# taufikxu/MOG-ASR

Hardware: AMD Instinct MI355X
Metric: images/sec/node AIR train step, Multi-MNIST 50×50 max_steps=3, 1/2/4/8 GPU (higher is better)
Workload: dtype fp32; 1 GPU; AIR baseline train step (training_air_original.py AIRModel, fp32), per-GPU batch 8192 (configs[1] batch); model=AIR (LSTM 256, VAE 784-512-256-50, heads 64), global_batch=8192, per_gpu_batch=8192, canvas=50x50, max_steps=3, data_dependent_steps_would_be=3, parallelism=dp1

## Files before the change

include/mog_air.h:

```cpp
#ifndef MOG_AIR_H
#define MOG_AIR_H

#ifdef __cplusplus
extern "C" {
#endif

#define MOG_ERR_INVALID 1001

int mog_gemm_f32(int batch, const float* const* A, const float* const* B, float* const* C,
                 const float* const* bias, const float* const* Cin, float* const* Cpre,
                 const float* const* aux, float* const* colsum, int M, int N, int K, int lda,
                 int ldb, int ldc, int ldaux, int transA, int transB, int epi, float aux_scale,
                 int splitk, void* stream);

int mog_gemm_f32_x3_tn(const float* A, const float* B, float* C, float* colsum, int M, int N,
                       int K, int lda, int ldb, int ldc, int splitk, float* work, long work_elems,
                       void* stream);

int mog_split3_bf16(const float* src, int rows, int cols, int ld_src, void* dst, int ld_dst,
                    long piece_stride, void* stream);
int mog_split3_sum_bf16(const float* src, int nsum, long sum_stride, int rows, int cols,
                        int ld_src, void* dst, int ld_dst, long piece_stride, void* stream);
int mog_gemm_x3p_tn(const void* A3, long sa, const void* B3, long sb, float* C, float* colsum,
                    int M, int N, int K, int lda, int ldb, int ldc, int splitk, int npieces,
// ... 1 lines not shown

int mog_build_id(char* out, int cap);

int mog_gemm_f32_wgrad_group(const long long* table, int nprob, void* stream);

long mog_wgrad_tn_work_elems(int nprob, const int* dims, int nsplit);
int mog_wgrad_tn_bf16(int nprob, const void* const* X, const void* const* dY, float* const* out,
                      float* const* colsum, const int* dims, int K, int nsplit, float* work,
                      long work_elems, void* stream);
int mog_wgrad_tn_x3(int nprob, const float* const* X, const float* const* dY, float* const* out,
                    float* const* colsum, const int* dims, int K, int nsplit, float* work,
                    long work_elems, void* stream);

int mog_gemm_x3_nt(const float* A, const void* B3, long sb, float* C, const float* aux, int M,
                   int N, int K, int lda, int ldb, int ldc, int ldaux, int epi, void* stream);

int mog_gemm_f32_sigmoid_philox(const float* A, const float* B, float* C, const float* bias,
                                int M, int N, int K, int lda, int ldb, int ldc, float scale,
                                unsigned long long seed, unsigned long long offset,
                                void* stream);
int mog_gemm_f32_kseg(int nseg, const float* const* A, const float* const* B, float* C,
                      const float* bias, const float* Cin, int M, int N, int kseg, int lda,
                      int ldb, int ldc, int transA, int transB, int epi, void* stream);
int mog_gemm_f32_kseg_group(int nprob, const int* nseg, const float* const* A,
                            const float* const* B, float* const* C, const float* const* Cin, int M,
                            int N, int kseg, int lda, int ldb, int ldc, int transB, void* stream);

int mog_stn_forward(const float* U, int N, int Hin, int Win, const float* theta, int Hout,
                    int Wout, void* out, const float* z, const float* mask, int mode,
                    void* stream);
// ... 238 lines not shown
```

mog-asr_amd/csrc/air_cell.hip:

```cpp
#include <algorithm>

#include "mog_common.h"

namespace {

struct LstmFwd {
  const float* G;
  const float* bias;
  const float* c_prev;
  float* c_out;
  float* h_out;
};

__device__ __forceinline__ void lstm_fwd_body(const LstmFwd& a, int B, int H, long idx) {
#pragma clang fp contract(off)
  if (idx >= (long)B * H) return;
  const int b = idx / H, u = idx - (long)b * H;
  const float* g = a.G + (size_t)b * 4 * H;
  float gi = g[u], gj = g[H + u], gf = g[2 * H + u], go = g[3 * H + u];
  if (a.bias) {
    const float* bias = a.bias;
    gi = gi + bias[u]; gj = gj + bias[H + u]; gf = gf + bias[2 * H + u]; go = go + bias[3 * H + u];
  }
  const float c0 = a.c_prev ? a.c_prev[idx] : 0.0f;
// ... 27 lines not shown
};

__device__ __forceinline__ void lstm_bwd_body(const LstmBwd& a, int B, int H, long idx) {
  if (idx >= (long)B * H) return;
  const int b = idx / H, u = idx - (long)b * H;
  const float* g = a.G + (size_t)b * 4 * H;
  const float* bp = a.bias ? a.bias : a.G;
  const float* cp = a.c_prev ? a.c_prev : a.c_cur;
  const float* dp = a.dc ? a.dc : a.dh;
  float* sp = a.dGsum ? a.dGsum + (size_t)b * 4 * H : a.dG + (size_t)b * 4 * H;
  float gi = g[u], gj = g[H + u], gf = g[2 * H + u], go = g[3 * H + u];
  const float bi = bp[u], bj = bp[H + u], bf = bp[2 * H + u], bo = bp[3 * H + u];
  const float cpv = cp[idx], ctv = a.c_cur[idx], dcv = dp[idx];
  float dhv = a.dh[idx];
  if (a.nparts > 0) {
    float pv[4];
#pragma unroll
    for (int j = 0; j < 4; ++j) pv[j] = j < a.nparts ? a.dh_parts[j * a.part_stride + idx] : 0.0f;
#pragma unroll
    for (int j = 0; j < 4; ++j)
      if (j < a.nparts) dhv = dhv + pv[j];
  }
  const float s0 = sp[u], s1 = sp[H + u], s2 = sp[2 * H + u], s3 = sp[3 * H + u];
  if (a.bias) {
    gi = gi + bi; gj = gj + bj; gf = gf + bf; go = go + bo;
  }
  const float si = mog_sigmoidf(gi), tj = mog_tanhf(gj), sf = mog_sigmoidf(gf + 1.0f);
  const float so = mog_sigmoidf(go);
  const float c0 = a.c_prev ? cpv : 0.0f;
  const float tc = mog_tanhf(ctv);
  const float dct = (a.dc ? dcv : 0.0f) + dhv * so * (1.0f - tc * tc);
  const float dgo = dhv * tc * so * (1.0f - so);
  const float dgf = dct * c0 * sf * (1.0f - sf);
  const float dgi = dct * tj * si * (1.0f - si);
  const float dgj = dct * si * (1.0f - tj * tj);
// ... 796 lines not shown
                                      float* dG, float* dc_prev, float* dGsum, int B, int H,
                                      void* stream) {
  MOG_CHECK_ARG(G && c_cur && dh && dG && B >= 0 && H > 0);
  if (B == 0) return 0;
  lstm_bwd_kernel<<<mog_cdiv((long)B * H, 256), 256, 0, mog_stream(stream)>>>(
      LstmBwd{G, bias, c_prev, c_cur, dh, dc, dG, dc_prev, dGsum}, B, H);
  MOG_LAUNCH_RET();
}

extern "C" int mog_lstm_cell_backward_parts(const float* G, const float* bias,
                                            const float* c_prev, const float* c_cur,
                                            const float* dh, const float* dh_parts, int nparts,
                                            long part_stride, const float* dc, float* dG,
                                            float* dc_prev, float* dGsum, int B, int H,
                                            void* stream) {
  MOG_CHECK_ARG(G && c_cur && dh && dG && B >= 0 && H > 0 && nparts >= 0 && nparts <= 4);
  MOG_CHECK_ARG(nparts == 0 || (dh_parts && part_stride >= (long)B * H));
  if (B == 0) return 0;
  LstmBwd a{G, bias, c_prev, c_cur, dh, dc, dG, dc_prev, dGsum};
  a.dh_parts = dh_parts;
  a.nparts = nparts;
  a.part_stride = part_stride;
  lstm_bwd_kernel<<<mog_cdiv((long)B * H, 256), 256, 0, mog_stream(stream)>>>(a, B, H);
  MOG_LAUNCH_RET();
}

extern "C" int mog_lstm_cell_forward_pair(const float* const* cells, int B, int H, void* stream) {
  MOG_CHECK_ARG(cells && B >= 0 && H > 0);
  const float* const* a = cells;
  const float* const* b = cells + 5;
  MOG_CHECK_ARG(a[0] && a[3] && a[4] && b[0] && b[3] && b[4]);
// ... 351 lines not shown
```

mog-asr_amd/csrc/gemm_x3.hip:

```cpp
#include <cstdlib>
#include <type_traits>

#include "mog_common.h"
#include "x3_split.h"

namespace {

typedef __bf16 bf16x8 __attribute__((ext_vector_type(8)));
typedef __bf16 bf16x4 __attribute__((ext_vector_type(4)));
typedef __attribute__((address_space(3))) bf16x4 lds_bf16x4;
typedef unsigned int u32x4 __attribute__((ext_vector_type(4)));

constexpr int BM = 128, BN = 128, BK = 32;
constexpr int LDR = BM;
constexpr int PIECE = BK * LDR;
constexpr int STAGE = 6 * PIECE;
constexpr int NL = (BM * BK / 4) / 256;

__device__ __forceinline__ int xcd_remap(int orig, int nwg) {
  const int xcd = orig & 7, q = nwg >> 3, r = nwg & 7;
  return (xcd < r ? xcd * (q + 1) : r * (q + 1) + (xcd - r) * q) + (orig >> 3);
}

__device__ __forceinline__ int tsw(int r) { return ((r & 3) << 2) | (((r >> 3) & 1) << 4); }
// ... 321 lines not shown
    float v = W[e];
    for (int s = 1; s < nsplit; ++s) v += W[s * MN + e];
    C[(size_t)(e / N) * ldc + e % N] += v;
  }
}

void splitk_reduce(const X3Args& D, hipStream_t s) {
  const long n4 = ((long)D.M * D.N + 3) / 4;
  const long nt = n4 > D.N ? n4 : (long)D.N;
  const bool vec = D.N % 4 == 0 && D.ldc % 4 == 0 && (reinterpret_cast<uintptr_t>(D.C) & 15) == 0;
  splitk_reduce_kernel<<<dim3((unsigned)((nt + 255) / 256)), 256, 0, s>>>(
      D.work, D.nsplit, D.C, D.M, D.N, D.ldc, vec, D.colsum);
}

constexpr int NT_LDK = BK + 16;
constexpr int NT_PIECE = BM * NT_LDK;
constexpr int NT_STAGE = 6 * NT_PIECE;
constexpr int NT_NLA = (BM * BK / 4) / 256;
constexpr int NT_NLB = (BN * BK / 8) / 256;

struct X3NtArgs {
  const float* A;
  const __bf16* B3;
  long sb;
  float* C;
  const float* aux;
  int M, N, K, lda, ldb, ldc, ldaux, nx, ny, epi;
};

__device__ __forceinline__ float xt_dpp1(float v) {
  return __int_as_float(__builtin_amdgcn_mov_dpp(__float_as_int(v), 0xB1, 0xF, 0xF, false));
}
__device__ __forceinline__ float xt_dpp2(float v) {
  return __int_as_float(__builtin_amdgcn_mov_dpp(__float_as_int(v), 0x4E, 0xF, 0xF, false));
}
__device__ __forceinline__ floatx4 xt_quad_transpose(const floatx4& a, int lane) {
  const int e = lane & 3;
  float r0 = a[0], r1 = a[1], r2 = a[2], r3 = a[3];
  {
    const bool hi = (e & 2) != 0;
    const float t0 = xt_dpp2(hi ? r0 : r2), t1 = xt_dpp2(hi ? r1 : r3);
    if (hi) { r0 = t0; r1 = t1; } else { r2 = t0; r3 = t1; }
  }
  {
    const bool od = (e & 1) != 0;
    const float t0 = xt_dpp1(od ? r0 : r1), t1 = xt_dpp1(od ? r2 : r3);
    if (od) { r0 = t0; r2 = t1; } else { r1 = t0; r3 = t1; }
  }
  return floatx4{r0, r1, r2, r3};
}

template <int EPI>
__global__ __launch_bounds__(256, 2) void gemm_x3_nt_kernel(X3NtArgs D) {
  __shared__ __attribute__((aligned(16))) __bf16 lds[NT_STAGE];
  const int nwg = gridDim.x;
  const int wg = xcd_remap(blockIdx.x, nwg);
  const int bx = wg % D.nx, by = wg / D.nx;
  const int m0 = by * BM, n0 = bx * BN;
  const int t = threadIdx.x, lane = t & 63, w = t >> 6;
  const int wm = (w >> 1) * 64, wn = (w & 1) * 64;
  const int M = D.M, N = D.N, K = D.K;
  const int ar = t >> 3, ak = (t & 7) * 4;
  const int br = t >> 2, bk = (t & 3) * 8;
  floatx4 acc[4][4];
#pragma unroll
  for (int mi = 0; mi < 4; ++mi)
#pragma unroll
    for (int ni = 0; ni < 4; ++ni) acc[mi][ni] = floatx4{0.f, 0.f, 0.f, 0.f};
  u32x4 ra[NT_NLA];
  u32x4 rb[3][NT_NLB];
  const int arows = min(M - m0, BM);
  const __amdgpu_buffer_rsrc_t arsc = __builtin_amdgcn_make_buffer_rsrc(
      const_cast<float*>(D.A) + (size_t)m0 * D.lda, 0,
      (M - m0 > BM ? BM * D.lda : (arows - 1) * D.lda + K) * 4, 0x00020000);
  __amdgpu_buffer_rsrc_t brsc[3];
#pragma unroll
  for (int p = 0; p < 3; ++p)
    brsc[p] = __builtin_amdgcn_make_buffer_rsrc(const_cast<__bf16*>(D.B3) + (size_t)p * D.sb, 0,
                                                ((N - 1) * D.ldb + K) * 2, 0x00020000);
  int avo[NT_NLA], bvo[NT_NLB];
#pragma unroll
  for (int i = 0; i < NT_NLA; ++i) avo[i] = ((ar + 32 * i) * D.lda + ak) * 4;
#pragma unroll
  for (int i = 0; i < NT_NLB; ++i) bvo[i] = ((n0 + br + 64 * i) * D.ldb + bk) * 2;
  constexpr int OOB = (int)0x80000000u;
  auto load_tiles = [&](int k0) {
    const bool ak_in = k0 + ak < K, bk_in = k0 + bk < K;
#pragma unroll
    for (int i = 0; i < NT_NLA; ++i)
      ra[i] = __builtin_amdgcn_raw_buffer_load_b128(arsc, ak_in ? avo[i] : OOB, k0 * 4, 0);
#pragma unroll
    for (int i = 0; i < NT_NLB; ++i)
#pragma unroll
      for (int p = 0; p < 3; ++p)
        rb[p][i] = __builtin_amdgcn_raw_buffer_load_b128(brsc[p], bk_in ? bvo[i] : OOB, k0 * 2, 0);
  };
  auto store_tiles = [&]() {
#pragma unroll
    for (int i = 0; i < NT_NLA; ++i) {
      const int o = (ar + 32 * i) * NT_LDK + ak;
      u32x2 p0, p1, p2;
      split4(float4{__uint_as_float(ra[i][0]), __uint_as_float(ra[i][1]),
                    __uint_as_float(ra[i][2]), __uint_as_float(ra[i][3])},
             p0, p1, p2);
      *reinterpret_cast<u32x2*>(lds + 0 * NT_PIECE + o) = p0;
      *reinterpret_cast<u32x2*>(lds + 1 * NT_PIECE + o) = p1;
      *reinterpret_cast<u32x2*>(lds + 2 * NT_PIECE + o) = p2;
    }
#pragma unroll
    for (int i = 0; i < NT_NLB; ++i) {
      const int o = (br + 64 * i) * NT_LDK + bk;
#pragma unroll
      for (int p = 0; p < 3; ++p) *reinterpret_cast<u32x4*>(lds + (3 + p) * NT_PIECE + o) = rb[p][i];
    }
  };
  const int g = lane >> 4, li = lane & 15;
  auto frag = [&](int piece, int row) -> bf16x8 {
    return *reinterpret_cast<const bf16x8*>(lds + piece * NT_PIECE + (row + li) * NT_LDK + 8 * g);
  };
  auto compute = [&]() {
    bf16x8 b[3][4];
#pragma unroll
    for (int p = 0; p < 3; ++p)
#pragma unroll
      for (int i = 0; i < 4; ++i) b[p][i] = frag(3 + p, wn + 16 * i);
    auto pass = [&](const bf16x8 (&x)[4], const bf16x8 (&y)[4]) {
#pragma unroll
      for (int mi = 0; mi < 4; ++mi)
#pragma unroll
        for (int ni = 0; ni < 4; ++ni)
          acc[mi][ni] = __builtin_amdgcn_mfma_f32_16x16x32_bf16(x[mi], y[ni], acc[mi][ni], 0, 0, 0);
    };
#pragma unroll
    for (int pa = 2; pa >= 0; --pa) {
      bf16x8 a[4];
#pragma unroll
      for (int i = 0; i < 4; ++i) a[i] = frag(pa, wm + 16 * i);
#pragma unroll
      for (int pb = 2 - pa; pb >= 0; --pb) pass(a, b[pb]);
    }
  };
  const int nk = (K + BK - 1) / BK;
  load_tiles(0);
  for (int it = 0; it < nk; ++it) {
    store_tiles();
    if (it + 1 < nk) load_tiles((it + 1) * BK);
    __syncthreads();
    compute();
    __syncthreads();
  }
  u32x4 xq[4][4];
  if constexpr (EPI == 1) {
    const __amdgpu_buffer_rsrc_t xr = __builtin_amdgcn_make_buffer_rsrc(
        const_cast<float*>(D.aux) + (size_t)m0 * D.ldaux, 0,
        (M - m0 > BM ? BM * D.ldaux : (arows - 1) * D.ldaux + N) * 4, 0x00020000);
#pragma unroll
    for (int mi = 0; mi < 4; ++mi)
#pragma unroll
      for (int ni = 0; ni < 4; ++ni)
        xq[mi][ni] = __builtin_amdgcn_raw_buffer_load_b128(
            xr, ((wm + mi * 16 + g * 4 + (li & 3)) * D.ldaux + n0 + wn + ni * 16 + (li & ~3)) * 4,
            0, 0);
  }
#pragma unroll
  for (int mi = 0; mi < 4; ++mi)
#pragma unroll
    for (int ni = 0; ni < 4; ++ni) {
      const floatx4 v = xt_quad_transpose(acc[mi][ni], lane);
      const int row = m0 + wm + mi * 16 + g * 4 + (li & 3);
      const int col = n0 + wn + ni * 16 + (li & ~3);
      float o[4] = {v[0], v[1], v[2], v[3]};
      if (EPI == 1) {
#pragma unroll
        for (int q = 0; q < 4; ++q) o[q] = v[q] * -mog_expm1f(-__uint_as_float(xq[mi][ni][q]));
      }
      if (row < M && col < N)
        *reinterpret_cast<float4*>(D.C + (size_t)row * D.ldc + col) = make_float4(o[0], o[1], o[2], o[3]);
    }
}

}

extern "C" int mog_split3_bf16(const float* src, int rows, int cols, int ld_src, void* dst,
                               int ld_dst, long piece_stride, void* stream) {
  MOG_CHECK_ARG(src && dst && rows >= 0 && cols >= 0 && cols % 4 == 0 && ld_src % 4 == 0 &&
                ld_dst % 4 == 0 && ld_dst >= cols && ld_src >= cols && piece_stride % 4 == 0 &&
                piece_stride >= (long)rows * ld_dst && al16(src) && al16(dst));
  const long n = (long)rows * (ld_dst / 4);
  if (n == 0) return 0;
  split3_kernel<<<dim3((unsigned)((n + 255) / 256)), 256, 0, mog_stream(stream)>>>(
      src, rows, cols, ld_src, reinterpret_cast<__bf16*>(dst), ld_dst, piece_stride);
  MOG_LAUNCH_RET();
}
// ... 53 lines not shown
}

extern "C" int mog_gemm_x3_nt(const float* A, const void* B3, long sb, float* C, const float* aux,
                              int M, int N, int K, int lda, int ldb, int ldc, int ldaux, int epi,
                              void* stream) {
  MOG_CHECK_ARG(A && B3 && C && M >= 0 && N >= 0 && K >= 0 && (epi == 0 || epi == 1));
  MOG_CHECK_ARG(epi == 0 || (aux && ldaux % 4 == 0 && ldaux >= N && al16(aux)));
  MOG_CHECK_ARG(al16(A) && al16(B3) && al16(C) && K % 8 == 0 && N % 4 == 0 && lda % 4 == 0 &&
                ldc % 4 == 0 && ldb % 8 == 0 && sb % 8 == 0 && lda >= K && ldb >= K && ldc >= N);
  MOG_CHECK_ARG((long)N * ldb * 2 < (1L << 31) && (long)BM * lda * 4 < (1L << 31) &&
                (long)BM * ldaux * 4 < (1L << 31));
  if (M == 0 || N == 0) return 0;
  X3NtArgs D{};
  D.A = A; D.B3 = reinterpret_cast<const __bf16*>(B3); D.sb = sb; D.C = C; D.aux = aux;
  D.M = M; D.N = N; D.K = K; D.lda = lda; D.ldb = ldb; D.ldc = ldc; D.ldaux = ldaux;
  D.nx = mog_cdiv(N, BN);
  D.ny = mog_cdiv(M, BM);
  D.epi = epi;
  const unsigned nwg = (unsigned)D.nx * D.ny;
  hipStream_t s = mog_stream(stream);
  if (epi == 1) gemm_x3_nt_kernel<1><<<nwg, 256, 0, s>>>(D);
  else gemm_x3_nt_kernel<0><<<nwg, 256, 0, s>>>(D);
  MOG_LAUNCH_RET();
}
```

mog-asr_amd/csrc/torch_ops.cpp:

```cpp
#include <ATen/ATen.h>
#include <ATen/hip/impl/HIPGuardImplMasqueradingAsCUDA.h>
#include <c10/hip/HIPStream.h>
#include <torch/library.h>

#include <vector>

#include "mog_air.h"

namespace {

using at::ScalarType;
using at::Tensor;
using c10::optional;
using std::vector;

constexpr ScalarType F32 = at::kFloat, BF16 = at::kBFloat16, I32 = at::kInt;

void check(int rc, const char* name) {
  TORCH_CHECK(rc == 0, "mog_air::", name, " failed: ",
              rc == MOG_ERR_INVALID ? "invalid argument" : "HIP error ", rc);
}

struct Op {
  const char* name;
// ... 1395 lines not shown
  check(mog_gemm_f32_wgrad_group(table.data(), (int)n, o.stream()), o.name);
}

void gemm_x3_nt_(const Tensor& A, const Tensor& B3, int64_t sb, Tensor C,
                 const optional<Tensor>& aux, int64_t M, int64_t N, int64_t K, int64_t lda,
                 int64_t ldb, int64_t ldc, int64_t ldaux, int64_t epi) {
  Op o("gemm_x3_nt_");
  float* c = o.f(C, mat(M, N, ldc), "C");
  const float* a = o.f(A, mat(M, K, lda), "A");
  const void* b = o.need(B3, BF16, 2 * sb + mat(N, ldb, ldb), "B3");
  const float* x = o.f(aux, mat(M, N, ldaux), "aux");
  GUARD(o);
  check(mog_gemm_x3_nt(a, b, sb, c, x, M, N, K, lda, ldb, ldc, ldaux, epi, o.stream()), o.name);
}

TORCH_LIBRARY_FRAGMENT(mog_air, m) {
  m.def(
      "gemm_x3_nt_(Tensor A, Tensor B3, int sb, Tensor(a!) C, Tensor? aux, int M, int N, int K, "
      "int lda, int ldb, int ldc, int ldaux, int epi) -> ()");
  m.def(
      "gemm_f32_wgrad_group_(Tensor[] X, Tensor[] dY, Tensor(a!)[] out, Tensor(b!)?[] bias, "
      "int[] dims) -> ()");
  m.def(
      "wgrad_tn_bf16_(Tensor[] X, Tensor[] dY, Tensor(a!)[] out, Tensor(b!)?[] colsum, int[] dims, "
      "int K, int nsplit) -> ()");
  m.def(
      "wgrad_tn_x3_(Tensor[] X, Tensor[] dY, Tensor(a!)[] out, Tensor(b!)?[] colsum, int[] dims, "
      "int K, int nsplit) -> ()");
  m.def(
      "split3_bf16_(Tensor src, Tensor(a!) dst, int rows, int cols, int ld_src, int ld_dst, "
      "int piece_stride) -> ()");
  m.def(
      "gemm_x3p_tn_(Tensor A3, int sa, Tensor B3, int sb, Tensor(a!) C, Tensor(b!)? colsum, "
      "int M, int N, int K, int lda, int ldb, int ldc, int splitk, int npieces=3, int reduce=1) -> ()");
// ... 194 lines not shown
      "Tensor? dss, Tensor(a!) douts, Tensor(b!)?[] dpre) -> ()");
  m.def(
      "asr_step_backward_learned_(int B, bool train, int fix_steps, float temperature, "
      "float grad_scale, Tensor[] w, Tensor[] gw, Tensor?[] hid, Tensor rec, Tensor eps_shift, "
      "Tensor eps_scale, Tensor dtheta_fwd, Tensor dtheta_back, Tensor dot, Tensor dreg, "
      "Tensor? dss, Tensor(a!) douts, Tensor(b!)?[] dpre) -> ()");
}

TORCH_LIBRARY_IMPL(mog_air, CUDA, m) {
  m.impl("gemm_f32_", &gemm_f32_);
  m.impl("gemm_f32_kseg_", &gemm_f32_kseg_);
  m.impl("gemm_f32_sigmoid_philox_", &gemm_f32_sigmoid_philox_);
  m.impl("gemm_f32_x3_tn_", &gemm_f32_x3_tn_);
  m.impl("split3_bf16_", &split3_bf16_);
  m.impl("gemm_x3_nt_", &gemm_x3_nt_);
  m.impl("gemm_x3p_tn_", &gemm_x3p_tn_);
  m.impl("gemm_f32_wgrad_group_", &gemm_f32_wgrad_group_);
  m.impl("wgrad_tn_bf16_", &wgrad_tn_bf16_);
  m.impl("wgrad_tn_x3_", &wgrad_tn_x3_);
  m.impl("gemm_bf16_", &gemm_bf16_);
  m.impl("cvt_bf16_batch_", &cvt_bf16_batch_);
  m.impl("stn_forward_", &stn_forward_);
  m.impl("stn_backward_", &stn_backward_);
  m.impl("stn_backward_sigmoid_", &stn_backward_sigmoid_);
  m.impl("lstm_cell_forward_", &lstm_cell_forward_);
  m.impl("lstm_cell_backward_", &lstm_cell_backward_);
  m.impl("gemm_f32_kseg_group_", &gemm_f32_kseg_group_);
  m.impl("lstm_cell_forward2_", &lstm_cell_forward2_);
  m.impl("lstm_cell_backward2_", &lstm_cell_backward2_);
  m.impl("heads_output_wgrad_", &heads_output_wgrad_);
// ... 41 lines not shown
```

mog-asr_amd/mog_air/_lib.py:

```python
from __future__ import annotations

import ctypes
import os
import re
from typing import List

_HERE = os.path.dirname(os.path.abspath(__file__))
LIB_PATH = os.environ.get("MOG_AIR_LIB") or os.path.join(_HERE, "_lib", "libmog_air.so")
HEADER_PATH = os.path.normpath(os.path.join(_HERE, "..", "..", "include", "mog_air.h"))

P = ctypes.c_void_p
I = ctypes.c_int
F = ctypes.c_float
L = ctypes.c_long
ULL = ctypes.c_ulonglong
LL = ctypes.c_longlong

_SIGS = {
    "mog_gemm_f32": [I, P, P, P, P, P, P, P, P, I, I, I, I, I, I, I, I, I, I, F, I, P],
    "mog_gemm_f32_kseg": [I, P, P, P, P, P, I, I, I, I, I, I, I, I, I, P],
    "mog_gemm_f32_x3_tn": [P, P, P, P, I, I, I, I, I, I, I, P, L, P],
    "mog_split3_bf16": [P, I, I, I, P, I, L, P],
    "mog_split3_sum_bf16": [P, I, L, I, I, I, P, I, L, P],
    "mog_gemm_x3p_tn": [P, L, P, L, P, P, I, I, I, I, I, I, I, I, P, L, P],
    "mog_gemm_f32_wgrad_group": [P, I, P],
    "mog_wgrad_tn_work_elems": [I, P, I],
    "mog_wgrad_tn_bf16": [I, P, P, P, P, P, I, I, P, L, P],
    "mog_wgrad_tn_x3": [I, P, P, P, P, P, I, I, P, L, P],
    "mog_build_id": [P, I],
    "mog_gemm_x3_nt": [P, P, L, P, P, I, I, I, I, I, I, I, I, P],
    "mog_gemm_f32_sigmoid_philox": [P, P, P, P, I, I, I, I, I, I, F, ULL, ULL, P],
    "mog_stn_forward": [P, I, I, I, P, I, I, P, P, P, I, P],
    "mog_stn_forward_periodic": [P, I, I, I, I, P, I, I, P, P, P, I, P],
    "mog_stn_backward": [P, I, I, I, P, I, I, P, P, P, P, P, I, I, P],
    "mog_stn_backward_sigmoid_bf16": [P, I, I, I, P, I, I, P, P, P, P, P, I, I, P],
    "mog_stn_backward_sigmoid_f32": [P, I, I, I, P, I, I, P, P, P, P, P, I, I, P],
    "mog_lstm_cell_forward": [P, P, P, P, P, I, I, P],
    "mog_lstm_cell_backward": [P, P, P, P, P, P, P, P, P, I, I, P],
    "mog_lstm_cell_backward_parts": [P, P, P, P, P, P, I, L, P, P, P, P, I, I, P],
    "mog_gemm_f32_kseg_group": [I, P, P, P, P, P, I, I, I, I, I, I, I, P],
    "mog_lstm_cell_forward_pair": [P, I, I, P],
    "mog_lstm_cell_backward_pair": [P, I, I, P],
    "mog_air_step_forward": [I, I, I, I, I, I, F, F, F, F, F, F, F, F, F, F, P, P, P, P, P, P,
                             P, P, P, P, P, P, P, P, P, P, P, P, P, P, P, P, P],
    "mog_air_step_forward_steps": [I, I, I, I, I, I, F, F, F, P, F, F, F, F, F, F, P, L, P, P, P,
# ... 186 lines not shown
```

mog-asr_amd/mog_air/air_model.py:

```python
from __future__ import annotations

import contextlib
from typing import Optional

import numpy as np
import torch

from . import ops
from .model_base import R_NREC, ModelBase, _Workspace, annealed_value
from .ops import EPI_RELU, gemm
from .params import CNN_LAYERS, cnn_param_specs, param_specs
from .results import Generation
from .wgrads import TALL_X3, WgradProblem

_ops = ops._ops

R_SM, R_SLV, R_HM0, R_HM1, R_HLV0, R_HLV1, R_LO, R_S, R_TX, R_TY, R_Y, R_Z = range(12)
R_ACT_OLD, R_ACT, R_LIVE, R_ZC, R_ZTERM = 12, 13, 14, 15, 16


def marginal_objective(num_prior, max_steps) -> np.ndarray:
    obj = np.zeros([max_steps])
    buf = 1.0 - 1.0 / len(num_prior)
    for ind in range(max_steps):
# ... 113 lines not shown
        Wx, Wh = K[:NX], K[NX:]
        Xl = self._cnn_forward(X, ws) if self.cnn else X
        side = self._side_stream() if ws.noise_side else None
        ws.noise_side = False
        if self.cnn and need_grad and self._x3p_xgrad(B):
            self._x_split3(Xl, ws)
        with torch.cuda.stream(side) if side is not None else contextlib.nullcontext():
            self._reset_loop_state(ws)
            if need_grad and self._x3p_xgrad(B) and not self.cnn:
                self._x_split3(X, ws)
            if need_grad and self.precision == "bf16":
                self._x_bf16(X, ws)
            if (need_grad and self.precision == "fp32" and self.VAE_DX_X3
                    and B * self.max_steps >= self.X3_DX_MIN_ROWS):
                self._w3()
            if side is not None:
                pre_done = torch.cuda.Event()
                pre_done.record(side)
        prior_lo = self.hyper("z_pres_prior_log_odds")
        temperature = self.hyper("z_pres_temperature")
        thr = self.hyper("stopping_threshold")
        lik_std = self.hyper("vae_likelihood_std")
        batched = self._batched_vae(B)
        with self._timed("lstm_x_projection"):
            gemm([Xl], [Wx], [ws.Gx], B, 4 * H, NX, NX, 4 * H, 4 * H)
        if side is not None:
            torch.cuda.current_stream().wait_event(pre_done)
        w1 = [self._P(h + "/hidden/weights") for h in self._HEADS]
        b1 = [self._P(h + "/hidden/biases") for h in self._HEADS]
        w2 = [self._P(h + "/output/weights") for h in self._HEADS]
# ... 117 lines not shown
                None, ws.rec, ws.eps_scale, ws.eps_shift, ws.dth_f_all, ws.dth_b_all, ws.dot_all,
                [ws.hid[z] for z in range(5)], w2, ws.dout[0], T * B * 2, ws.dhid, HS,
                self._prior_arg(), T)
        for t in range(T if self.marginal is not None else 0):
            hid_t = [ws.hid[z, t] for z in range(5)]
            _ops.air_step_backward_(
                B, HS, self.train, self.marginal is not None, temperature, prior_lo,
                float(self.marginal[t]) if self.marginal is not None else 0.0,
                float(self.scale_prior_mean), float(self.scale_prior_variance),
                float(self.shift_prior_mean), float(self.shift_prior_variance), float(gscale),
                None, ws.rec[t], ws.eps_scale[t], ws.eps_shift[t], ws.dth_f_all[t], ws.dth_b_all[t],
                ws.dot_all[t], hid_t, w2, ws.dout[0, t], T * B * 2, ws.dhid[t], HS,
                self._prior_arg())
        if w1_done is not None:
            torch.cuda.current_stream().wait_event(w1_done)
        if B < self.SIDE_MIN_BATCH and HS % 16 == 0:
            dhid = ws.dhid.view(TB, 5 * HS)
            ops.gemm_kseg([dhid[:, z * HS:] for z in range(5)],
                          [self._P(h + "/hidden/weights") for h in self._HEADS], ws.dh, TB, H,
                          HS, 5 * HS, HS, H, transB=True)
        else:
            gemm([ws.dhid], [self._w1cat()], [ws.dh], TB, H, 5 * HS, 5 * HS, 5 * HS, H,
                 transB=True)
        heads_side = (self.grad_reducer is None and self.HEADS_WGRAD_SIDE
                      and B >= self.SIDE_MIN_BATCH)
        if heads_side:
            with torch.cuda.stream(self._fork(self._stream3())):
                self._weight_grads_heads(ws)
        else:
            self._weight_grads_heads(ws)
            if vae_done is not None:
                torch.cuda.current_stream().wait_event(vae_done)
            split = self._bucket_split()
            self._reduce_bucket(split, self.params.total)
        rec_early = T > 1 and heads_side and self.REC_WGRAD_SIDE
        dGsum = None if self._x3p_xgrad(B) and not self.cnn else ws.dGsum
        parts = self._dh_parts(B)
        dh_parts = ws.buffer("dh_parts", (parts, B, H)) if parts else None
        for t in reversed(range(T)):
            dc_in = ws.dc[(t + 1) % 2] if t < T - 1 else None
            G_t, b_t = (ws.Gx, bK) if t == 0 else (ws.G[t], None)
            c_prev = ws.c[t - 1] if t > 0 else None
            if parts and t < T - 1:
                _ops.lstm_cell_backward_parts_(G_t, b_t, c_prev, ws.c[t], ws.dh[t], dh_parts,
                                               parts, dc_in, ws.dG[t], ws.dc[t % 2], dGsum, B, H)
            else:
                _ops.lstm_cell_backward_(G_t, b_t, c_prev, ws.c[t], ws.dh[t], dc_in, ws.dG[t],
                                         ws.dc[t % 2], dGsum, B, H)
            if t == 1 and rec_early:
                self._weight_grads_rec_side(ws)
            if t > 0 and parts:
                kp = 4 * H // parts
                gemm([ws.dG[t][:, j * kp:] for j in range(parts)],
                     [Wh[:, j * kp:] for j in range(parts)], [dh_parts[j] for j in range(parts)],
                     B, H, kp, 4 * H, 4 * H, H, transB=True)
            elif t > 0:
                gemm([ws.dG[t]], [Wh], [ws.dh[t - 1]], B, H, 4 * H, 4 * H, 4 * H, H,
                     transB=True, Cin=[ws.dh[t - 1]])
        self._weight_grads_lstm(ws.feat if self.cnn else X, ws, side=heads_side,
                                rec_done=rec_early)
        if self.cnn:
            gemm([ws.dGsum], [Wx], [ws.dF], B, self.lstm_in, 4 * H, 4 * H, 4 * H, self.lstm_in,
                 transB=True)
            with self._timed("cnn_enc_backward"):
                ops.cnn_enc_backward(X, self._cnn_tensors(), ws.pool1, ws.pool2, ws.feat, ws.dF,
                                     ws.cnn_part, self._cnn_tensors("grad"))
        if heads_side:
            torch.cuda.current_stream().wait_stream(self._side_stream())
            torch.cuda.current_stream().wait_stream(self._stream3())

    HEADS_WGRAD_SIDE = True
    REC_WGRAD_SIDE = True

    def _w1cat(self):
        return self._wcache.get("w1cat", self._w1cat_build)

    def _w1cat_build(self):
        buf = torch.empty((self.rnn_units, 5 * self.scale_hidden_units), device=self.device)
        return buf, lambda: torch.cat([self._P(h + "/hidden/weights") for h in self._HEADS],
                                      dim=1, out=buf)

    def _weight_grads_heads(self, ws):
        H, HS, TB = self.rnn_units, self.scale_hidden_units, ws.B * self.max_steps
        heads = list(enumerate(self._HEADS))
        dhid = ws.dhid.view(TB, 5, HS)
        g = self._G
        cols = [2 if h.startswith("shift") else 1 for _, h in heads]
        hidden = [WgradProblem(ws.h, dhid[:, zi], g(h + "/hidden/weights"),
                               g(h + "/hidden/biases"), H, HS, H, 5 * HS) for zi, h in heads]
        plan = self._wgrads(hidden, TB, "heads_wgrad_x3", tall=HS < 128, group_first=True)
        if plan[0].form == TALL_X3:
            _ops.heads_output_wgrad_([ws.hid[zi] for zi, _ in heads],
                                     [ws.dout[zi] for zi, _ in heads],
                                     [g(h + "/output/weights") for _, h in heads],
                                     [g(h + "/output/biases") for _, h in heads], cols, TB, HS)
# ... 45 lines not shown
```

mog-asr_amd/mog_air/model_base.py:

```python
from __future__ import annotations

import contextlib
from typing import Dict, Optional

import numpy as np
import torch

from . import _lib
from . import ops
from .graph import GraphCapture
from .params import ParamStore, WeightCache
from .results import Results
from .vae import GlimpseVAE
from .wgrads import WeightGradients

_ops = ops._ops

R_NREC = 17

_SCOPES: Dict[str, ParamStore] = {}


def _f32log(v: float) -> float:
    return float(np.log(np.float32(v), dtype=np.float32))
# ... 350 lines not shown

    def _stn_write_backward_all(self, ws) -> None:
        TB, C = self.max_steps * ws.B, self.canvas_size
        dm = ws.dmb if self.precision == "bf16" else ws.dm
        ops.stn_backward(ws.r.view(TB, -1), ws.th_b, (C, C), ws.dcanvas, gscale=ws.zc,
                         dtheta=ws.dth_b_all, dot=ws.dot_all, want_dot=True, n=TB,
                         dm=dm.view(TB, -1))

    DH_PARTS = 4
    SIDE_MIN_BATCH = 1024

    def _dh_parts(self, B: int) -> int:
        return self.DH_PARTS if (B < self.SIDE_MIN_BATCH and self.DH_PARTS > 1
                                 and (4 * self.rnn_units) % (4 * self.DH_PARTS) == 0) else 0

    def _stn_bwd_work(self, rows, write):
        W2, C2, T = self.W2, self.C2, self.max_steps
        if write:
            dm = 2 if self.precision == "bf16" else 4
            return ("hbm", rows * (W2 * 4 + W2 * dm + C2 * 4 / T + 52), None)
        return ("hbm", rows * (C2 * 4 / T + W2 * 4 + 48), None)

    def _stream3(self):
        return _shared_streams(self.device)[1]

    def _side_stream(self):
        return _shared_streams(self.device)[0]

    SPIN_FORK = 0
    SPIN_MAIN = 0
# ... 65 lines not shown
```

mog-asr_amd/mog_air/ops.py:

```python
from __future__ import annotations

from typing import Optional, Sequence

import torch

from . import _lib

_lib.load_torch_ops()
_ops = torch.ops.mog_air

EPI_STORE, EPI_RELU, EPI_SOFTPLUS, EPI_SIGMOID_NOISE = 0, 1, 2, 3
EPI_SOFTPLUS_BWD, EPI_ATOMIC, EPI_RELU_BWD = 4, 5, 6


def stream_ptr() -> int:
    return torch.cuda.current_stream().cuda_stream


def dp(t: Optional[torch.Tensor]):
    if t is None:
        return None
    return t.data_ptr()


# ... 31 lines not shown
                ld_dst: int, piece_stride: int) -> None:
    _ops.split3_bf16_(src, dst, rows, cols, ld_src, ld_dst, int(piece_stride))


def gemm_x3p_tn(A3: torch.Tensor, sa: int, B3: torch.Tensor, sb: int, C: torch.Tensor, M: int,
                N: int, K: int, lda: int, ldb: int, ldc: int, splitk: int = 8,
                colsum=None, npieces: int = 3, reduce: bool = True) -> None:
    _ops.gemm_x3p_tn_(A3, int(sa), B3, int(sb), C, colsum, M, N, K, lda, ldb, ldc, int(splitk),
                      int(npieces), int(reduce))


def gemm_x3_nt(A: torch.Tensor, B3: torch.Tensor, sb: int, C: torch.Tensor, M: int, N: int,
               K: int, lda: int, ldb: int, ldc: int, aux=None, ldaux: int = 0) -> None:
    _ops.gemm_x3_nt_(A, B3, int(sb), C, aux, M, N, K, lda, ldb, ldc, int(ldaux),
                     1 if aux is not None else 0)


def wgrad_tn_bf16(X: Sequence[torch.Tensor], dY: Sequence[torch.Tensor],
                  out: Sequence[torch.Tensor], colsum: Sequence[Optional[torch.Tensor]],
                  dims: Sequence[Sequence[int]], K: int, nsplit: int = 8) -> None:
    _ops.wgrad_tn_bf16_(list(X), list(dY), list(out), list(colsum),
                        [int(d) for ds in dims for d in ds], int(K), int(nsplit))


def wgrad_tn_x3(X: Sequence[torch.Tensor], dY: Sequence[torch.Tensor],
                out: Sequence[torch.Tensor], colsum: Sequence[Optional[torch.Tensor]],
                dims: Sequence[Sequence[int]], K: int, nsplit: int = 8) -> None:
    _ops.wgrad_tn_x3_(list(X), list(dY), list(out), list(colsum),
                      [int(d) for ds in dims for d in ds], int(K), int(nsplit))

# ... 245 lines not shown
```

Measured before the change: 2.863 million images/sec.

## Route LSTM and heads dh backward GEMMs through batched bf16x3 MFMA kernel

Adds a batched variant of the bf16x3-split NT GEMM, with a selectable 64 or 128 M-tile, and uses it for the heads hidden-gradient GEMM and the per-timestep LSTM recurrent dh GEMM when the batch is large (B>=8192). The recurrent weights and concatenated head weights are pre-split into three bf16 pieces and cached. The LSTM dh GEMM is split along K into two partial outputs, which the LSTM backward cell sums; that cell now accepts up to 8 parts. This replaces the fp32 GEMM paths with emulated-fp32 matrix-core math, trading extra split and cache work and slight numeric differences for higher matrix throughput.

After: 2.883 million images/sec (median of 6 runs). Within noise of the previous version (+0.7%).

```diff
diff --git a/include/mog_air.h b/include/mog_air.h
--- a/include/mog_air.h
+++ b/include/mog_air.h
@@ -39,6 +39,9 @@
 
 int mog_gemm_x3_nt(const float* A, const void* B3, long sb, float* C, const float* aux, int M,
                    int N, int K, int lda, int ldb, int ldc, int ldaux, int epi, void* stream);
+int mog_gemm_x3_nt_batch(const float* A, long bsa, const void* B3, long sb, long bsb, float* C,
+                         long bsc, int nbatch, int M, int N, int K, int lda, int ldb, int ldc,
+                         int tile, void* stream);
 
 int mog_gemm_f32_sigmoid_philox(const float* A, const float* B, float* C, const float* bias,
                                 int M, int N, int K, int lda, int ldb, int ldc, float scale,
diff --git a/mog-asr_amd/csrc/air_cell.hip b/mog-asr_amd/csrc/air_cell.hip
--- a/mog-asr_amd/csrc/air_cell.hip
+++ b/mog-asr_amd/csrc/air_cell.hip
@@ -65,11 +65,11 @@
   const float cpv = cp[idx], ctv = a.c_cur[idx], dcv = dp[idx];
   float dhv = a.dh[idx];
   if (a.nparts > 0) {
-    float pv[4];
-#pragma unroll
-    for (int j = 0; j < 4; ++j) pv[j] = j < a.nparts ? a.dh_parts[j * a.part_stride + idx] : 0.0f;
-#pragma unroll
-    for (int j = 0; j < 4; ++j)
+    float pv[8];
+#pragma unroll
+    for (int j = 0; j < 8; ++j) pv[j] = j < a.nparts ? a.dh_parts[j * a.part_stride + idx] : 0.0f;
+#pragma unroll
+    for (int j = 0; j < 8; ++j)
       if (j < a.nparts) dhv = dhv + pv[j];
   }
   const float s0 = sp[u], s1 = sp[H + u], s2 = sp[2 * H + u], s3 = sp[3 * H + u];
@@ -896,7 +896,7 @@
                                             long part_stride, const float* dc, float* dG,
                                             float* dc_prev, float* dGsum, int B, int H,
                                             void* stream) {
-  MOG_CHECK_ARG(G && c_cur && dh && dG && B >= 0 && H > 0 && nparts >= 0 && nparts <= 4);
+  MOG_CHECK_ARG(G && c_cur && dh && dG && B >= 0 && H > 0 && nparts >= 0 && nparts <= 8);
   MOG_CHECK_ARG(nparts == 0 || (dh_parts && part_stride >= (long)B * H));
   if (B == 0) return 0;
   LstmBwd a{G, bias, c_prev, c_cur, dh, dc, dG, dc_prev, dGsum};
diff --git a/mog-asr_amd/csrc/gemm_x3.hip b/mog-asr_amd/csrc/gemm_x3.hip
--- a/mog-asr_amd/csrc/gemm_x3.hip
+++ b/mog-asr_amd/csrc/gemm_x3.hip
@@ -359,9 +359,7 @@
 }
 
 constexpr int NT_LDK = BK + 16;
-constexpr int NT_PIECE = BM * NT_LDK;
-constexpr int NT_STAGE = 6 * NT_PIECE;
-constexpr int NT_NLA = (BM * BK / 4) / 256;
+constexpr int NT_BPIECE = BN * NT_LDK;
 constexpr int NT_NLB = (BN * BK / 8) / 256;
 
 struct X3NtArgs {
@@ -371,6 +369,7 @@
   float* C;
   const float* aux;
   int M, N, K, lda, ldb, ldc, ldaux, nx, ny, epi;
+  long bsa, bsb, bsc;
 };
 
 __device__ __forceinline__ float xt_dpp1(float v) {
@@ -395,33 +394,41 @@
   return floatx4{r0, r1, r2, r3};
 }
 
-template <int EPI>
+template <int EPI, int TM>
 __global__ __launch_bounds__(256, 2) void gemm_x3_nt_kernel(X3NtArgs D) {
-  __shared__ __attribute__((aligned(16))) __bf16 lds[NT_STAGE];
+  constexpr int MI = TM / 32;
+  constexpr int NT_APIECE = TM * NT_LDK;
+  constexpr int NT_NLA = (TM * BK / 4) / 256;
+  __shared__ __attribute__((aligned(16))) __bf16 lds[3 * NT_APIECE + 3 * NT_BPIECE];
+  __bf16* const ldsb = lds + 3 * NT_APIECE;
   const int nwg = gridDim.x;
   const int wg = xcd_remap(blockIdx.x, nwg);
-  const int bx = wg % D.nx, by = wg / D.nx;
-  const int m0 = by * BM, n0 = bx * BN;
+  const int per = D.nx * D.ny, mem = wg / per, tile = wg - mem * per;
+  const int bx = tile % D.nx, by = tile / D.nx;
+  const int m0 = by * TM, n0 = bx * BN;
   const int t = threadIdx.x, lane = t & 63, w = t >> 6;
-  const int wm = (w >> 1) * 64, wn = (w & 1) * 64;
+  const int wm = (w >> 1) * (TM / 2), wn = (w & 1) * 64;
   const int M = D.M, N = D.N, K = D.K;
+  const float* const Am = D.A + (size_t)mem * D.bsa;
+  const __bf16* const Bm = D.B3 + (size_t)mem * D.bsb;
+  float* const Cm = D.C + (size_t)mem * D.bsc;
   const int ar = t >> 3, ak = (t & 7) * 4;
   const int br = t >> 2, bk = (t & 3) * 8;
-  floatx4 acc[4][4];
-#pragma unroll
-  for (int mi = 0; mi < 4; ++mi)
+  floatx4 acc[MI][4];
+#pragma unroll
+  for (int mi = 0; mi < MI; ++mi)
 #pragma unroll
     for (int ni = 0; ni < 4; ++ni) acc[mi][ni] = floatx4{0.f, 0.f, 0.f, 0.f};
   u32x4 ra[NT_NLA];
   u32x4 rb[3][NT_NLB];
-  const int arows = min(M - m0, BM);
+  const int arows = min(M - m0, TM);
   const __amdgpu_buffer_rsrc_t arsc = __builtin_amdgcn_make_buffer_rsrc(
-      const_cast<float*>(D.A) + (size_t)m0 * D.lda, 0,
-      (M - m0 > BM ? BM * D.lda : (arows - 1) * D.lda + K) * 4, 0x00020000);
+      const_cast<float*>(Am) + (size_t)m0 * D.lda, 0,
+      (M - m0 > TM ? TM * D.lda : (arows - 1) * D.lda + K) * 4, 0x00020000);
   __amdgpu_buffer_rsrc_t brsc[3];
 #pragma unroll
   for (int p = 0; p < 3; ++p)
-    brsc[p] = __builtin_amdgcn_make_buffer_rsrc(const_cast<__bf16*>(D.B3) + (size_t)p * D.sb, 0,
+    brsc[p] = __builtin_amdgcn_make_buffer_rsrc(const_cast<__bf16*>(Bm) + (size_t)p * D.sb, 0,
                                                 ((N - 1) * D.ldb + K) * 2, 0x00020000);
   int avo[NT_NLA], bvo[NT_NLB];
 #pragma unroll
@@ -448,39 +455,39 @@
       split4(float4{__uint_as_float(ra[i][0]), __uint_as_float(ra[i][1]),
                     __uint_as_float(ra[i][2]), __uint_as_float(ra[i][3])},
              p0, p1, p2);
-      *reinterpret_cast<u32x2*>(lds + 0 * NT_PIECE + o) = p0;
-      *reinterpret_cast<u32x2*>(lds + 1 * NT_PIECE + o) = p1;
-      *reinterpret_cast<u32x2*>(lds + 2 * NT_PIECE + o) = p2;
+      *reinterpret_cast<u32x2*>(lds + 0 * NT_APIECE + o) = p0;
+      *reinterpret_cast<u32x2*>(lds + 1 * NT_APIECE + o) = p1;
+      *reinterpret_cast<u32x2*>(lds + 2 * NT_APIECE + o) = p2;
     }
 #pragma unroll
     for (int i = 0; i < NT_NLB; ++i) {
       const int o = (br + 64 * i) * NT_LDK + bk;
 #pragma unroll
-      for (int p = 0; p < 3; ++p) *reinterpret_cast<u32x4*>(lds + (3 + p) * NT_PIECE + o) = rb[p][i];
+      for (int p = 0; p < 3; ++p) *reinterpret_cast<u32x4*>(ldsb + p * NT_BPIECE + o) = rb[p][i];
     }
   };
   const int g = lane >> 4, li = lane & 15;
-  auto frag = [&](int piece, int row) -> bf16x8 {
-    return *reinterpret_cast<const bf16x8*>(lds + piece * NT_PIECE + (row + li) * NT_LDK + 8 * g);
+  auto frag = [&](const __bf16* P, int row) -> bf16x8 {
+    return *reinterpret_cast<const bf16x8*>(P + (row + li) * NT_LDK + 8 * g);
   };
   auto compute = [&]() {
     bf16x8 b[3][4];
 #pragma unroll
     for (int p = 0; p < 3; ++p)
 #pragma unroll
-      for (int i = 0; i < 4; ++i) b[p][i] = frag(3 + p, wn + 16 * i);
-    auto pass = [&](const bf16x8 (&x)[4], const bf16x8 (&y)[4]) {
-#pragma unroll
-      for (int mi = 0; mi < 4; ++mi)
+      for (int i = 0; i < 4; ++i) b[p][i] = frag(ldsb + p * NT_BPIECE, wn + 16 * i);
+    auto pass = [&](const bf16x8 (&x)[MI], const bf16x8 (&y)[4]) {
+#pragma unroll
+      for (int mi = 0; mi < MI; ++mi)
 #pragma unroll
         for (int ni = 0; ni < 4; ++ni)
           acc[mi][ni] = __builtin_amdgcn_mfma_f32_16x16x32_bf16(x[mi], y[ni], acc[mi][ni], 0, 0, 0);
     };
 #pragma unroll
     for (int pa = 2; pa >= 0; --pa) {
-      bf16x8 a[4];
-#pragma unroll
-      for (int i = 0; i < 4; ++i) a[i] = frag(pa, wm + 16 * i);
+      bf16x8 a[MI];
+#pragma unroll
+      for (int i = 0; i < MI; ++i) a[i] = frag(lds + pa * NT_APIECE, wm + 16 * i);
 #pragma unroll
       for (int pb = 2 - pa; pb >= 0; --pb) pass(a, b[pb]);
     }
@@ -494,13 +501,13 @@
     compute();
     __syncthreads();
   }
-  u32x4 xq[4][4];
+  u32x4 xq[MI][4];
   if constexpr (EPI == 1) {
     const __amdgpu_buffer_rsrc_t xr = __builtin_amdgcn_make_buffer_rsrc(
         const_cast<float*>(D.aux) + (size_t)m0 * D.ldaux, 0,
-        (M - m0 > BM ? BM * D.ldaux : (arows - 1) * D.ldaux + N) * 4, 0x00020000);
-#pragma unroll
-    for (int mi = 0; mi < 4; ++mi)
+        (M - m0 > TM ? TM * D.ldaux : (arows - 1) * D.ldaux + N) * 4, 0x00020000);
+#pragma unroll
+    for (int mi = 0; mi < MI; ++mi)
 #pragma unroll
       for (int ni = 0; ni < 4; ++ni)
         xq[mi][ni] = __builtin_amdgcn_raw_buffer_load_b128(
@@ -508,7 +515,7 @@
             0, 0);
   }
 #pragma unroll
-  for (int mi = 0; mi < 4; ++mi)
+  for (int mi = 0; mi < MI; ++mi)
 #pragma unroll
     for (int ni = 0; ni < 4; ++ni) {
       const floatx4 v = xt_quad_transpose(acc[mi][ni], lane);
@@ -520,8 +527,22 @@
         for (int q = 0; q < 4; ++q) o[q] = v[q] * -mog_expm1f(-__uint_as_float(xq[mi][ni][q]));
       }
       if (row < M && col < N)
-        *reinterpret_cast<float4*>(D.C + (size_t)row * D.ldc + col) = make_float4(o[0], o[1], o[2], o[3]);
-    }
+        *reinterpret_cast<float4*>(Cm + (size_t)row * D.ldc + col) = make_float4(o[0], o[1], o[2], o[3]);
+    }
+}
+
+int nt_tile(int M, int N, int nbatch) {
+  const long wg128 = (long)mog_cdiv(M, 128) * mog_cdiv(N, BN) * nbatch;
+  return wg128 < 256 ? 64 : 128;
+}
+
+void launch_x3_nt(X3NtArgs D, int nbatch, int tile, hipStream_t s) {
+  D.nx = mog_cdiv(D.N, BN);
+  D.ny = mog_cdiv(D.M, tile);
+  const unsigned nwg = (unsigned)D.nx * D.ny * nbatch;
+  if (tile == 64) gemm_x3_nt_kernel<0, 64><<<nwg, 256, 0, s>>>(D);
+  else if (D.epi == 1) gemm_x3_nt_kernel<1, 128><<<nwg, 256, 0, s>>>(D);
+  else gemm_x3_nt_kernel<0, 128><<<nwg, 256, 0, s>>>(D);
 }
 
 }
@@ -605,12 +626,27 @@
   X3NtArgs D{};
   D.A = A; D.B3 = reinterpret_cast<const __bf16*>(B3); D.sb = sb; D.C = C; D.aux = aux;
   D.M = M; D.N = N; D.K = K; D.lda = lda; D.ldb = ldb; D.ldc = ldc; D.ldaux = ldaux;
-  D.nx = mog_cdiv(N, BN);
-  D.ny = mog_cdiv(M, BM);
   D.epi = epi;
-  const unsigned nwg = (unsigned)D.nx * D.ny;
-  hipStream_t s = mog_stream(stream);
-  if (epi == 1) gemm_x3_nt_kernel<1><<<nwg, 256, 0, s>>>(D);
-  else gemm_x3_nt_kernel<0><<<nwg, 256, 0, s>>>(D);
+  launch_x3_nt(D, 1, 128, mog_stream(stream));
   MOG_LAUNCH_RET();
 }
+
+extern "C" int mog_gemm_x3_nt_batch(const float* A, long bsa, const void* B3, long sb, long bsb,
+                                    float* C, long bsc, int nbatch, int M, int N, int K, int lda,
+                                    int ldb, int ldc, int tile, void* stream) {
+  MOG_CHECK_ARG(A && B3 && C && M >= 0 && N >= 0 && K >= 0 && nbatch >= 1 &&
+                (tile == 0 || tile == 64 || tile == 128));
+  MOG_CHECK_ARG(al16(A) && al16(B3) && al16(C) && K % 8 == 0 && N % 4 == 0 && lda % 4 == 0 &&
+                ldc % 4 == 0 && ldb % 8 == 0 && sb % 8 == 0 && lda >= K && ldb >= K && ldc >= N &&
+                bsa >= 0 && bsb >= 0 && bsc >= 0 && bsa % 4 == 0 && bsb % 8 == 0 && bsc % 4 == 0);
+  MOG_CHECK_ARG(nbatch == 1 || M == 0 || N == 0 || bsc >= (long)(M - 1) * ldc + N);
+  MOG_CHECK_ARG((long)N * ldb * 2 < (1L << 31) && (long)BM * lda * 4 < (1L << 31) &&
+                (long)nbatch * mog_cdiv(N, BN) * mog_cdiv(M, 64) < (1L << 31));
+  if (M == 0 || N == 0) return 0;
+  X3NtArgs D{};
+  D.A = A; D.B3 = reinterpret_cast<const __bf16*>(B3); D.sb = sb; D.C = C;
+  D.M = M; D.N = N; D.K = K; D.lda = lda; D.ldb = ldb; D.ldc = ldc;
+  D.bsa = bsa; D.bsb = bsb; D.bsc = bsc;
+  launch_x3_nt(D, nbatch, tile ? tile : nt_tile(M, N, nbatch), mog_stream(stream));
+  MOG_LAUNCH_RET();
+}
diff --git a/mog-asr_amd/csrc/torch_ops.cpp b/mog-asr_amd/csrc/torch_ops.cpp
--- a/mog-asr_amd/csrc/torch_ops.cpp
+++ b/mog-asr_amd/csrc/torch_ops.cpp
@@ -1433,10 +1433,28 @@
   check(mog_gemm_x3_nt(a, b, sb, c, x, M, N, K, lda, ldb, ldc, ldaux, epi, o.stream()), o.name);
 }
 
+void gemm_x3_nt_batch_(const Tensor& A, int64_t bsa, const Tensor& B3, int64_t sb, int64_t bsb,
+                       Tensor C, int64_t bsc, int64_t nbatch, int64_t M, int64_t N, int64_t K,
+                       int64_t lda, int64_t ldb, int64_t ldc, int64_t tile) {
+  Op o("gemm_x3_nt_batch_");
+  TORCH_CHECK(nbatch >= 1 && bsa >= 0 && bsb >= 0 && bsc >= 0 && sb >= 0, o.name,
+              ": nbatch >= 1 and non-negative strides");
+  float* c = o.f(C, (nbatch - 1) * bsc + mat(M, N, ldc), "C");
+  const float* a = o.f(A, (nbatch - 1) * bsa + mat(M, K, lda), "A");
+  const void* b = o.need(B3, BF16, 2 * sb + (nbatch - 1) * bsb + mat(N, K, ldb), "B3");
+  GUARD(o);
+  check(mog_gemm_x3_nt_batch(a, bsa, b, sb, bsb, c, bsc, (int)nbatch, M, N, K, lda, ldb, ldc,
+                             (int)tile, o.stream()),
+        o.name);
+}
+
 TORCH_LIBRARY_FRAGMENT(mog_air, m) {
   m.def(
       "gemm_x3_nt_(Tensor A, Tensor B3, int sb, Tensor(a!) C, Tensor? aux, int M, int N, int K, "
       "int lda, int ldb, int ldc, int ldaux, int epi) -> ()");
+  m.def(
+      "gemm_x3_nt_batch_(Tensor A, int bsa, Tensor B3, int sb, int bsb, Tensor(a!) C, int bsc, "
+      "int nbatch, int M, int N, int K, int lda, int ldb, int ldc, int tile) -> ()");
   m.def(
       "gemm_f32_wgrad_group_(Tensor[] X, Tensor[] dY, Tensor(a!)[] out, Tensor(b!)?[] bias, "
       "int[] dims) -> ()");
@@ -1661,6 +1679,7 @@
   m.impl("gemm_f32_x3_tn_", &gemm_f32_x3_tn_);
   m.impl("split3_bf16_", &split3_bf16_);
   m.impl("gemm_x3_nt_", &gemm_x3_nt_);
+  m.impl("gemm_x3_nt_batch_", &gemm_x3_nt_batch_);
   m.impl("gemm_x3p_tn_", &gemm_x3p_tn_);
   m.impl("gemm_f32_wgrad_group_", &gemm_f32_wgrad_group_);
   m.impl("wgrad_tn_bf16_", &wgrad_tn_bf16_);
diff --git a/mog-asr_amd/mog_air/_lib.py b/mog-asr_amd/mog_air/_lib.py
--- a/mog-asr_amd/mog_air/_lib.py
+++ b/mog-asr_amd/mog_air/_lib.py
@@ -29,6 +29,7 @@
     "mog_wgrad_tn_x3": [I, P, P, P, P, P, I, I, P, L, P],
     "mog_build_id": [P, I],
     "mog_gemm_x3_nt": [P, P, L, P, P, I, I, I, I, I, I, I, I, P],
+    "mog_gemm_x3_nt_batch": [P, L, P, L, L, P, L, I, I, I, I, I, I, I, I, P],
     "mog_gemm_f32_sigmoid_philox": [P, P, P, P, I, I, I, I, I, I, F, ULL, ULL, P],
     "mog_stn_forward": [P, I, I, I, P, I, I, P, P, P, I, P],
     "mog_stn_forward_periodic": [P, I, I, I, I, P, I, I, P, P, P, I, P],
diff --git a/mog-asr_amd/mog_air/air_model.py b/mog-asr_amd/mog_air/air_model.py
--- a/mog-asr_amd/mog_air/air_model.py
+++ b/mog-asr_amd/mog_air/air_model.py
@@ -151,6 +151,8 @@
             if (need_grad and self.precision == "fp32" and self.VAE_DX_X3
                     and B * self.max_steps >= self.X3_DX_MIN_ROWS):
                 self._w3()
+            if need_grad and self._dh_x3(B):
+                self._dh_w3()
             if side is not None:
                 pre_done = torch.cuda.Event()
                 pre_done.record(side)
@@ -298,7 +300,12 @@
                 self._prior_arg())
         if w1_done is not None:
             torch.cuda.current_stream().wait_event(w1_done)
-        if B < self.SIDE_MIN_BATCH and HS % 16 == 0:
+        x3_parts = self._dh_x3(B)
+        if x3_parts and TB >= self.X3_DX_MIN_ROWS and (5 * HS) % 8 == 0:
+            with self._timed("heads_dh_x3", ("mfma", 2.0 * TB * H * 5 * HS, "fp32", "x3")):
+                ops.gemm_x3_nt_batch(ws.dhid, 0, self._dh_w3()[1], H * 5 * HS, 0, ws.dh, 0, 1, TB,
+                                     H, 5 * HS, 5 * HS, 5 * HS, H, tile=self.DH_X3_TILE)
+        elif B < self.SIDE_MIN_BATCH and HS % 16 == 0:
             dhid = ws.dhid.view(TB, 5 * HS)
             ops.gemm_kseg([dhid[:, z * HS:] for z in range(5)],
                           [self._P(h + "/hidden/weights") for h in self._HEADS], ws.dh, TB, H,
@@ -319,8 +326,11 @@
             self._reduce_bucket(split, self.params.total)
         rec_early = T > 1 and heads_side and self.REC_WGRAD_SIDE
         dGsum = None if self._x3p_xgrad(B) and not self.cnn else ws.dGsum
-        parts = self._dh_parts(B)
+        parts = x3_parts or self._dh_parts(B)
+        if parts and ws.dh_parts is not None and ws.dh_parts.shape[0] != parts:
+            ws.dh_parts = None
         dh_parts = ws.buffer("dh_parts", (parts, B, H)) if parts else None
+        wh3 = self._dh_w3()[0] if x3_parts and T > 1 else None
         for t in reversed(range(T)):
             dc_in = ws.dc[(t + 1) % 2] if t < T - 1 else None
             G_t, b_t = (ws.Gx, bK) if t == 0 else (ws.G[t], None)
@@ -333,7 +343,12 @@
                                          ws.dc[t % 2], dGsum, B, H)
             if t == 1 and rec_early:
                 self._weight_grads_rec_side(ws)
-            if t > 0 and parts:
+            if t > 0 and x3_parts:
+                kp = 4 * H // parts
+                with self._timed("lstm_dh_x3", ("mfma", 2.0 * B * H * 4 * H, "fp32", "x3")):
+                    ops.gemm_x3_nt_batch(ws.dG[t], kp, wh3, H * 4 * H, kp, dh_parts, B * H, parts,
+                                         B, H, kp, 4 * H, 4 * H, H, tile=self.DH_X3_TILE)
+            elif t > 0 and parts:
                 kp = 4 * H // parts
                 gemm([ws.dG[t][:, j * kp:] for j in range(parts)],
                      [Wh[:, j * kp:] for j in range(parts)], [dh_parts[j] for j in range(parts)],
@@ -363,6 +378,20 @@
         buf = torch.empty((self.rnn_units, 5 * self.scale_hidden_units), device=self.device)
         return buf, lambda: torch.cat([self._P(h + "/hidden/weights") for h in self._HEADS],
                                       dim=1, out=buf)
+
+    def _dh_w3(self):
+        return self._wcache.get("dh_w3", self._dh_w3_build)
+
+    def _dh_w3_build(self):
+        H, HS = self.rnn_units, self.scale_hidden_units
+        wh3 = torch.empty((3, H, 4 * H), device=self.device, dtype=torch.bfloat16)
+        w13 = torch.empty((3, H, 5 * HS), device=self.device, dtype=torch.bfloat16)
+
+        def refresh():
+            Wh = self._P("rnn/basic_lstm_cell/kernel")[self.lstm_in:]
+            ops.split3_bf16(Wh, wh3, H, 4 * H, 4 * H, 4 * H, H * 4 * H)
+            ops.split3_bf16(self._w1cat(), w13, H, 5 * HS, 5 * HS, 5 * HS, H * 5 * HS)
+        return (wh3, w13), refresh
 
     def _weight_grads_heads(self, ws):
         H, HS, TB = self.rnn_units, self.scale_hidden_units, ws.B * self.max_steps
diff --git a/mog-asr_amd/mog_air/model_base.py b/mog-asr_amd/mog_air/model_base.py
--- a/mog-asr_amd/mog_air/model_base.py
+++ b/mog-asr_amd/mog_air/model_base.py
@@ -388,6 +388,17 @@
         return self.DH_PARTS if (B < self.SIDE_MIN_BATCH and self.DH_PARTS > 1
                                  and (4 * self.rnn_units) % (4 * self.DH_PARTS) == 0) else 0
 
+    DH_X3 = True
+    DH_X3_MIN_B = 8192
+    DH_X3_PARTS = 2
+    DH_X3_TILE = 0
+
+    def _dh_x3(self, B: int) -> int:
+        p, H = self.DH_X3_PARTS, self.rnn_units
+        ok = (self.DH_X3 and self.precision == "fp32" and B >= self.DH_X3_MIN_B
+              and 1 <= p <= 8 and H % 4 == 0 and (4 * H) % (8 * p) == 0)
+        return p if ok else 0
+
     def _stn_bwd_work(self, rows, write):
         W2, C2, T = self.W2, self.C2, self.max_steps
         if write:
diff --git a/mog-asr_amd/mog_air/ops.py b/mog-asr_amd/mog_air/ops.py
--- a/mog-asr_amd/mog_air/ops.py
+++ b/mog-asr_amd/mog_air/ops.py
@@ -69,6 +69,13 @@
                K: int, lda: int, ldb: int, ldc: int, aux=None, ldaux: int = 0) -> None:
     _ops.gemm_x3_nt_(A, B3, int(sb), C, aux, M, N, K, lda, ldb, ldc, int(ldaux),
                      1 if aux is not None else 0)
+
+
+def gemm_x3_nt_batch(A: torch.Tensor, bsa: int, B3: torch.Tensor, sb: int, bsb: int,
+                     C: torch.Tensor, bsc: int, nbatch: int, M: int, N: int, K: int, lda: int,
+                     ldb: int, ldc: int, tile: int = 0) -> None:
+    _ops.gemm_x3_nt_batch_(A, int(bsa), B3, int(sb), int(bsb), C, int(bsc), int(nbatch), M, N, K,
+                           lda, ldb, ldc, int(tile))
 
 
 def wgrad_tn_bf16(X: Sequence[torch.Tensor], dY: Sequence[torch.Tensor],
```
